# sjappig/rtl-ws

Hardware: AMD Instinct MI355X
Metric: spectra/s (1024-pt IQ frames) (higher is better)
Workload: dtype f64 arithmetic, f32 rows; 1 GPU; batched_1024pt_64k_frames_f64c_f32o; n_fft=1024, k_avg=1, window=rect, output=power_sum, cic_r=0, input=cmplx_u8 tone(0.6)+noise(0.05), device-resident, 4 rotating sets

## Files before the change

### rtl-ws_amd/csrc/spectrum_f64_1024x.hip

```cpp
#include <hip/hip_runtime.h>
#include <stdint.h>

#include "rtlws_internal.h"
#include "fft_regs_f64.h"

#define RTLWS_X_LDS_ORDER 0

namespace rtlws {

using namespace f64;

typedef short pk_i16 __attribute__((ext_vector_type(2)));

__device__ __forceinline__ void swap_rows16(unsigned& a, unsigned& b)
{
    const auto r = __builtin_amdgcn_permlane16_swap(a, b, false, false);
    a = r[0];
    b = r[1];
}
__device__ __forceinline__ void swap_rows32(unsigned& a, unsigned& b)
{
    const auto r = __builtin_amdgcn_permlane32_swap(a, b, false, false);
    a = r[0];
    b = r[1];
}

template <int OUT, bool KONE, bool ROWF32, int WAVES>
__global__ __launch_bounds__(64 * WAVES, WAVES == 1 ? 2 : WAVES / 4) void spectra_f64_1024x(const SpectraParamsF64 p)
{
    constexpr int N = 1024;
    static_assert(!(ROWF32 && OUT == OUT_PAYLOAD), "payload rows are bytes in either form");
    static_assert(WAVES == 1 || WAVES % 4 == 0, "whole wavefronts per SIMD");
    extern __shared__ __attribute__((aligned(16))) double2 lds_all[];
    constexpr int SLICE_F2 = 17 * 64;
    double2* const ldsd = lds_all + (WAVES == 1 ? 0 : (threadIdx.x >> 6) * SLICE_F2);
    unsigned* const row_counter = reinterpret_cast<unsigned*>(lds_all + WAVES * SLICE_F2);

    const int t = threadIdx.x & 63;
    const int K = KONE ? 1 : p.k_avg;
    const long ngroups = p.ngroups;
    long g = (long)blockIdx.x + (WAVES == 1 ? 0L : (long)(threadIdx.x >> 6) * gridDim.x);
    if constexpr (WAVES > 1) {
        if (threadIdx.x == 0) *row_counter = WAVES;
        __syncthreads();
    }
    auto next_row = [&](long cur) -> long {
        if constexpr (WAVES == 1) {
            return cur + gridDim.x;
        } else {
            unsigned v = 0;
            if (t == 0) v = __hip_atomic_fetch_add(row_counter, 1u, __ATOMIC_RELAXED, __HIP_MEMORY_SCOPE_WORKGROUP);
            return (long)blockIdx.x + (long)(unsigned)__builtin_amdgcn_readfirstlane((int)v) * gridDim.x;
        }
    };

    unsigned raw[16];
    auto load_raw = [&](long frame) {
        const uint16_t* src = reinterpret_cast<const uint16_t*>(p.in) + frame * N;
#pragma unroll
        for (int j = 0; j < 16; ++j) raw[j] = __builtin_nontemporal_load(src + 64 * j + t);
    };
    if (g < ngroups) load_raw(g * K);

    f2 twA[8], twB[16];
#pragma unroll
    for (int m = 0; m < 8; ++m) twA[m] = p.twxa[(t >> 4) * 8 + m];
#pragma unroll
    for (int s = 0; s < 16; ++s) twB[s] = p.twxb[t * 16 + s];
#pragma unroll
    for (int m = 0; m < 8; ++m) asm volatile("" ::"v"(twA[m].x), "v"(twA[m].y));
#pragma unroll
    for (int s = 0; s < 16; ++s) asm volatile("" ::"v"(twB[s].x), "v"(twB[s].y));

    const int wp = t >> 4, wc = t & 15;

    while (g < ngroups) {
        const long g_next = next_row(g);
        double acc[16];
        double wdc = 0.0;
#pragma unroll
        for (int u = 0; u < 16; ++u) acc[u] = 0.0;

        for (int kf = 0; kf < K; ++kf) {
            const long frame = g * K + kf;

            unsigned y[16];
#pragma unroll
            for (int b = 0; b < 4; ++b) {
                pk_i16 x[4];
#pragma unroll
                for (int a = 0; a < 4; ++a) {
                    const unsigned r = raw[4 * a + b];
                    x[a] = __builtin_bit_cast(pk_i16, __builtin_amdgcn_perm(r, r, 0x0c010c00u));
                }
                const pk_i16 s0 = x[0] + x[2], s1 = x[0] - x[2], s2 = x[1] + x[3], s3 = x[1] - x[3];
                const pk_i16 rot = {s3.y, (short)-s3.x};
                y[4 * b + 0] = __builtin_bit_cast(unsigned, (pk_i16)(s0 + s2));
                y[4 * b + 1] = __builtin_bit_cast(unsigned, (pk_i16)(s1 + rot));
                y[4 * b + 2] = __builtin_bit_cast(unsigned, (pk_i16)(s0 - s2));
                y[4 * b + 3] = __builtin_bit_cast(unsigned, (pk_i16)(s1 - rot));
            }
            {
                long nf = frame + 1;
                if (kf + 1 == K) nf = g_next * K;
                if (nf >= ngroups * K) nf = frame;
                load_raw(nf);
            }

#pragma unroll
            for (int b = 0; b < 4; ++b) {
                swap_rows16(y[4 * b + 0], y[4 * b + 1]);
                swap_rows16(y[4 * b + 2], y[4 * b + 3]);
                swap_rows32(y[4 * b + 0], y[4 * b + 2]);
                swap_rows32(y[4 * b + 1], y[4 * b + 3]);
            }
            f2 v[16];
#pragma unroll
            for (int r = 0; r < 16; ++r)
                v[r] = mk((double)(short)(y[r] & 0xffffu), (double)((int)y[r] >> 16));

            fft_last<16>(v, 0, twA);
#pragma unroll
            for (int s = 0; s < 16; ++s) v[s] = cmul(v[s], twB[s]);

            __builtin_amdgcn_fence(__ATOMIC_RELEASE, "wavefront");
            __builtin_amdgcn_wave_barrier();
#pragma unroll
            for (int s = 0; s < 16; ++s) ldsd[17 * (4 * rev16(s) + wp) + wc] = v[s];
            __builtin_amdgcn_fence(__ATOMIC_RELEASE, "wavefront");
            __builtin_amdgcn_wave_barrier();
            __builtin_amdgcn_fence(__ATOMIC_ACQUIRE, "wavefront");
#pragma unroll
            for (int c = 0; c < 16; ++c) v[c] = ldsd[17 * t + c];

            fft16_sel(v);

#pragma unroll
            for (int u = 0; u < 16; ++u) {
                if (u == 15) {
                    const double pw = fma(v[u].y, v[u].y, v[u].x * v[u].x);
                    acc[u] = KONE ? pw : acc[u] + pw;
                    wdc = KONE ? pw : fma((double)(K - kf), pw, wdc);
                } else if constexpr (KONE) {
                    acc[u] = fma(v[u].y, v[u].y, v[u].x * v[u].x);
                } else {
                    acc[u] = fma(v[u].y, v[u].y, fma(v[u].x, v[u].x, acc[u]));
                }
            }
        }

        const double dcv = lane63(wdc);
        if (t == 0) acc[0] = dcv;

        {
#pragma unroll
            for (int u = 0; u < 16; ++u) {
                const long i = g * N + 64 * (rev16(u) ^ 8) + t;
                const double a = acc[u];
                if constexpr (OUT == OUT_PAYLOAD) {
                    reinterpret_cast<uint8_t*>(p.out)[i] = (uint8_t)payload_f64(p.lin_gain * a, p.count);
                } else {
                    const double o = (OUT == OUT_DB) ? db_f64(a, p.count) : a;
                    if constexpr (ROWF32) __builtin_nontemporal_store((float)o, reinterpret_cast<float*>(p.out) + i);
                    else __builtin_nontemporal_store(o, reinterpret_cast<double*>(p.out) + i);
                }
            }
        }
        g = g_next;
    }
}

constexpr size_t x_lds_bytes(int waves) { return (size_t)waves * 16 * 17 * 64 + (waves > 1 ? 16 : 0); }
size_t spectra_f64_1024x_lds_bytes(int waves) { return x_lds_bytes(waves >= 8 ? 8 : 1); }

template <typename Choose, typename Leaf>
static hipError_t x_table(Choose choose, const SpectraParamsF64& p, int waves, Leaf&& leaf)
{
    return choose(Vals<1, 8>{}, waves >= 8 ? 8 : 1, [&](auto w) {
        return choose(OutModes{}, p.out_mode, [&](auto out) {
            using Kone = std::conditional_t<out == OUT_SUM, Bools, Vals<true>>;
            return choose(Kone{}, p.k_avg == 1, [&](auto kone) {
                return choose(Flag<out != OUT_PAYLOAD>{}, p.rows_f32 != 0, [&](auto rowf32) {
                    return leaf(&spectra_f64_1024x<out, kone, rowf32, w>, 64 * w, x_lds_bytes(w));
                });
            });
        });
    });
}

hipError_t launch_spectra_f64_1024x(const SpectraParamsF64& p, int blocks, int waves, hipStream_t st, int device)
{
    return x_table(pick, p, waves, [&](auto kernel, int threads, size_t lds_bytes) {
        const hipError_t e = lds_opt_in(kernel, device, lds_bytes);
        return e != hipSuccess ? e : launch(kernel, dim3(blocks), dim3(threads), lds_bytes, st, p);
    });
}

hipError_t prepare_spectra_f64_1024x(int device)
{
    return x_table(visit_all, SpectraParamsF64{}, 0, [&](auto kernel, int, size_t lds_bytes) {
        return lds_opt_in(kernel, device, lds_bytes);
    });
}

}
```

Measured before the change: 587.4 million spectra/s.

## Compute first radix-4 FFT stage with int8 MFMA instead of packed-int VALU

For the k_avg==1 path, the first radix-4 butterfly over the u8 IQ samples becomes an i8 16x16x32 MFMA against a constant ±1 coefficient matrix. The u8 samples are sign-flipped to s8, and the removed offset is restored through a DC term in the accumulator. This replaces the byte unpacking, packed-i16 adds and permlane row swaps, because the matrix layout yields the transposed result directly. In exchange it adds byte-granular load packing, 8 MFMA issues per frame and a sched_barrier, and correctness depends on the MFMA lane layout matching the expected data placement.

Measured after the change: 623.8 million spectra/s (median of 6 runs). 1.06x the previous value.

```diff
diff --git a/rtl-ws_amd/csrc/spectrum_f64_1024x.hip b/rtl-ws_amd/csrc/spectrum_f64_1024x.hip
--- a/rtl-ws_amd/csrc/spectrum_f64_1024x.hip
+++ b/rtl-ws_amd/csrc/spectrum_f64_1024x.hip
@@ -11,6 +11,20 @@
 using namespace f64;
 
 typedef short pk_i16 __attribute__((ext_vector_type(2)));
+typedef unsigned short pk_u16 __attribute__((ext_vector_type(2)));
+typedef int v4i __attribute__((ext_vector_type(4)));
+
+constexpr long radix4_coef(int p, bool im)
+{
+    unsigned long v = 0;
+    for (int a = 0; a < 4; ++a) {
+        const int e = (a * p) & 3;
+        const int cr = e == 0 ? 1 : e == 2 ? -1 : 0, ci = e == 1 ? -1 : e == 3 ? 1 : 0;
+        v |= (unsigned long)(unsigned char)(im ? ci : cr) << (16 * a);
+        v |= (unsigned long)(unsigned char)(im ? cr : -ci) << (16 * a + 8);
+    }
+    return (long)v;
+}
 
 __device__ __forceinline__ void swap_rows16(unsigned& a, unsigned& b)
 {
@@ -54,13 +68,36 @@
         }
     };
 
-    unsigned raw[16];
+    constexpr bool MFMA_FE = KONE;
+    unsigned raw[MFMA_FE ? 8 : 16];
     auto load_raw = [&](long frame) {
         const uint16_t* src = reinterpret_cast<const uint16_t*>(p.in) + frame * N;
-#pragma unroll
-        for (int j = 0; j < 16; ++j) raw[j] = __builtin_nontemporal_load(src + 64 * j + t);
+        if constexpr (MFMA_FE) {
+#pragma unroll
+            for (int b = 0; b < 4; ++b) {
+#pragma unroll
+                for (int h = 0; h < 2; ++h) {
+                    pk_u16 w;
+                    w.x = __builtin_nontemporal_load(src + 64 * (8 * h + b) + t);
+                    w.y = __builtin_nontemporal_load(src + 64 * (8 * h + 4 + b) + t);
+                    raw[2 * b + h] = __builtin_bit_cast(unsigned, w);
+                }
+            }
+        } else {
+#pragma unroll
+            for (int j = 0; j < 16; ++j) raw[j] = __builtin_nontemporal_load(src + 64 * j + t);
+        }
     };
     if (g < ngroups) load_raw(g * K);
+
+    long a_re = 0, a_im = 0;
+    if ((t >> 4) == (t & 3)) {
+        const int pp = (t & 15) >> 2;
+        a_re = pp == 0 ? radix4_coef(0, false) : pp == 1 ? radix4_coef(1, false) : pp == 2 ? radix4_coef(2, false) : radix4_coef(3, false);
+        a_im = pp == 0 ? radix4_coef(0, true) : pp == 1 ? radix4_coef(1, true) : pp == 2 ? radix4_coef(2, true) : radix4_coef(3, true);
+    }
+    const int c_dc = t < 16 ? 512 : 0;
+    const v4i c_off = {c_dc, c_dc, c_dc, c_dc};
 
     f2 twA[8], twB[16];
 #pragma unroll
@@ -84,40 +121,56 @@
         for (int kf = 0; kf < K; ++kf) {
             const long frame = g * K + kf;
 
-            unsigned y[16];
-#pragma unroll
-            for (int b = 0; b < 4; ++b) {
-                pk_i16 x[4];
-#pragma unroll
-                for (int a = 0; a < 4; ++a) {
-                    const unsigned r = raw[4 * a + b];
-                    x[a] = __builtin_bit_cast(pk_i16, __builtin_amdgcn_perm(r, r, 0x0c010c00u));
-                }
-                const pk_i16 s0 = x[0] + x[2], s1 = x[0] - x[2], s2 = x[1] + x[3], s3 = x[1] - x[3];
-                const pk_i16 rot = {s3.y, (short)-s3.x};
-                y[4 * b + 0] = __builtin_bit_cast(unsigned, (pk_i16)(s0 + s2));
-                y[4 * b + 1] = __builtin_bit_cast(unsigned, (pk_i16)(s1 + rot));
-                y[4 * b + 2] = __builtin_bit_cast(unsigned, (pk_i16)(s0 - s2));
-                y[4 * b + 3] = __builtin_bit_cast(unsigned, (pk_i16)(s1 - rot));
-            }
-            {
+            auto prefetch = [&]() {
                 long nf = frame + 1;
                 if (kf + 1 == K) nf = g_next * K;
                 if (nf >= ngroups * K) nf = frame;
                 load_raw(nf);
-            }
-
-#pragma unroll
-            for (int b = 0; b < 4; ++b) {
-                swap_rows16(y[4 * b + 0], y[4 * b + 1]);
-                swap_rows16(y[4 * b + 2], y[4 * b + 3]);
-                swap_rows32(y[4 * b + 0], y[4 * b + 2]);
-                swap_rows32(y[4 * b + 1], y[4 * b + 3]);
-            }
+            };
             f2 v[16];
-#pragma unroll
-            for (int r = 0; r < 16; ++r)
-                v[r] = mk((double)(short)(y[r] & 0xffffu), (double)((int)y[r] >> 16));
+            if constexpr (MFMA_FE) {
+                v4i yre[4], yim[4];
+#pragma unroll
+                for (int b = 0; b < 4; ++b) {
+                    const unsigned lo = raw[2 * b] ^ 0x80808080u, hi = raw[2 * b + 1] ^ 0x80808080u;
+                    const long xb = (long)(((unsigned long)hi << 32) | lo);
+                    yre[b] = __builtin_amdgcn_mfma_i32_16x16x32_i8(a_re, xb, c_off, 0, 0, 0);
+                    yim[b] = __builtin_amdgcn_mfma_i32_16x16x32_i8(a_im, xb, c_off, 0, 0, 0);
+                }
+                __builtin_amdgcn_sched_barrier(0);
+                prefetch();
+#pragma unroll
+                for (int r = 0; r < 16; ++r) v[r] = mk((double)yre[r >> 2][r & 3], (double)yim[r >> 2][r & 3]);
+            } else {
+                unsigned y[16];
+#pragma unroll
+                for (int b = 0; b < 4; ++b) {
+                    pk_i16 x[4];
+#pragma unroll
+                    for (int a = 0; a < 4; ++a) {
+                        const unsigned r = raw[4 * a + b];
+                        x[a] = __builtin_bit_cast(pk_i16, __builtin_amdgcn_perm(r, r, 0x0c010c00u));
+                    }
+                    const pk_i16 s0 = x[0] + x[2], s1 = x[0] - x[2], s2 = x[1] + x[3], s3 = x[1] - x[3];
+                    const pk_i16 rot = {s3.y, (short)-s3.x};
+                    y[4 * b + 0] = __builtin_bit_cast(unsigned, (pk_i16)(s0 + s2));
+                    y[4 * b + 1] = __builtin_bit_cast(unsigned, (pk_i16)(s1 + rot));
+                    y[4 * b + 2] = __builtin_bit_cast(unsigned, (pk_i16)(s0 - s2));
+                    y[4 * b + 3] = __builtin_bit_cast(unsigned, (pk_i16)(s1 - rot));
+                }
+                prefetch();
+
+#pragma unroll
+                for (int b = 0; b < 4; ++b) {
+                    swap_rows16(y[4 * b + 0], y[4 * b + 1]);
+                    swap_rows16(y[4 * b + 2], y[4 * b + 3]);
+                    swap_rows32(y[4 * b + 0], y[4 * b + 2]);
+                    swap_rows32(y[4 * b + 1], y[4 * b + 3]);
+                }
+#pragma unroll
+                for (int r = 0; r < 16; ++r)
+                    v[r] = mk((double)(short)(y[r] & 0xffffu), (double)((int)y[r] >> 16));
+            }
 
             fft_last<16>(v, 0, twA);
 #pragma unroll
```
